# DanielPS555/Radix-sort-Merge-Sort-CUDA---Lab-y-practicos-GPGPU-2023

Hardware: NVIDIA B200
Metric: 32-bit keys sorted/sec at n=2^28 (higher is better)
Workload: dtype int32

## Files before the change

### radix-sort-merge-sort-cuda---lab-y-practicos-gpgpu-2023_b200/csrc/radix.cu

```cuda
#include "radix.cuh"
#include "radix_hist.cuh"
#include "radix_tile.cuh"
#include "radix_pipelined.cuh"
#include "radix_tma.cuh"
#include "radix_tma2.cuh"
#include "radix_tma3.cuh"
#include "radix_misc.cuh"
#include "radix_small.cuh"

#include <atomic>
#include <cstdlib>
#include <mutex>

namespace b200sort {

__global__ void __launch_bounds__(kSmallThreads, 1)
radix_small_kernel(const int32_t *in, int32_t *out, uint32_t n)
{
    radix_small_body<0>(in, out, n, SignXor{0x80000000u, 0x80000000u});
}
__global__ void __launch_bounds__(kSmallThreads, 1)
radix_small_keys_kernel(const int32_t *in, int32_t *out, uint32_t n, SignXor order)
{
    radix_small_body<1>(in, out, n, order);
}

namespace {

using OnesweepFn = void (*)(const int32_t *, int32_t *, int32_t *, size_t, int, RadixControl *,
                            uint32_t *, uint32_t *, int);

struct Variant {
    const char *name;
    int mode;
    int cluster;
    int two_level;
    int threads;
    int tile;
    size_t smem;
// ... 238 lines not shown
    const size_t chunks = div_up(div_up(n, 4), (size_t)kHistThreads * kHistUnroll);
    size_t g = chunks < (size_t)kNumSMs * kHistBlocksPerSM ? chunks : (size_t)kNumSMs * kHistBlocksPerSM;
    return (int)(g < 1 ? 1 : g);
}

}

namespace {
int effective_variant() {
    const int v = g_variant.load();
    if (kVariants[v].mode == kRankAdd && !atomic_order_ok()) return kFallbackVariant;
    return v;
}
}

int radix_set_phase_debug(long long *d_buf) {
    B200_CUDA_TRY(cudaMemcpyToSymbol(g_phase_dbg, &d_buf, sizeof d_buf));
    return B200SORT_OK;
}
int radix_atomic_order_ok() { return atomic_order_ok(); }
unsigned long long radix_check_failures(unsigned long long *per_site) { return tu_check_failures(per_site); }
int radix_num_variants() { return kNumVariants; }
const char *radix_variant_name(int v) { return (v >= 0 && v < kNumVariants) ? kVariants[v].name : nullptr; }
int radix_set_variant(int v) {
    if (v < 0 || v >= kNumVariants) return B200SORT_ERR_INVALID;
    g_variant.store(v);
    g_small_enabled.store((v == 0 && g_small_env_on) ? 1 : 0);
    return B200SORT_OK;
}
void radix_set_skip(int enabled) { g_skip_enabled.store(enabled ? 1 : 0); }
size_t radix_current_tile() { return (size_t)kVariants[g_variant.load()].tile; }
const char *radix_effective_variant_name() { return kVariants[effective_variant()].name; }

size_t radix_workspace_bytes(size_t n) {
    const size_t tiles = div_up(n > 0 ? n : 1, kRadixMinTile);
    const size_t rows = tiles + div_up(tiles, (size_t)kPPGroup) + 1;
    return kRadixControlBytes + 2 * rows * kRadixBins * sizeof(uint32_t);
}

int radix_histogram(const int32_t *d_keys, size_t n, uint32_t *d_hist, cudaStream_t s) {
    RadixControl *scratch = nullptr;
    B200_CUDA_TRY(cudaMallocAsync(reinterpret_cast<void **>(&scratch), kRadixControlBytes, s));
    int rc = ensure_hist_attr();
    if (rc == B200SORT_OK) rc = record_cuda(cudaMemsetAsync(scratch, 0, kRadixZeroBytes, s));
    if (rc == B200SORT_OK && n > 0) {
        radix_histogram_kernel<<<hist_grid(n), kHistThreads, kHistSmemBytes, s>>>(d_keys, n, scratch, nullptr, 0, 0, 0);
        ++g_launch_count;
        rc = record_cuda(cudaGetLastError());
    }
    if (rc == B200SORT_OK)
        rc = record_cuda(cudaMemcpyAsync(d_hist, scratch->hist, sizeof(uint32_t) * kRadixPasses * kRadixBins,
                                         cudaMemcpyDeviceToDevice, s));
    cudaFreeAsync(scratch, s);
    return rc;
}

static int check_ws(void *d_ws, size_t ws_bytes, size_t n) {
    if (d_ws == nullptr || (reinterpret_cast<uintptr_t>(d_ws) & 255) != 0) return B200SORT_ERR_WORKSPACE;
    if (ws_bytes < radix_workspace_bytes(n)) return B200SORT_ERR_WORKSPACE;
    return B200SORT_OK;
}

int radix_single_pass(const int32_t *d_in, int32_t *d_out, size_t n, int pass, void *d_ws,
                      size_t ws_bytes, cudaStream_t s) {
    if (pass < 0 || pass >= kRadixPasses) return B200SORT_ERR_INVALID;
    if (n == 0) return B200SORT_OK;
    B200_TRY(check_ws(d_ws, ws_bytes, n));
    const int v = effective_variant();
    B200_TRY(ensure_smem_attr(v));
    B200_TRY(ensure_hist_attr());
// ... 50 lines not shown
        if (order != nullptr) {
            B200_CUDA_TRY(cudaFuncSetAttribute(reinterpret_cast<const void *>(radix_small_keys_kernel),
                                               cudaFuncAttributeMaxDynamicSharedMemorySize, (int)kSmallSmemBytes));
            radix_small_keys_kernel<<<1, kSmallThreads, kSmallSmemBytes, s>>>(d_in, d_out, (uint32_t)n, *order);
        } else {
            B200_CUDA_TRY(cudaFuncSetAttribute(reinterpret_cast<const void *>(radix_small_kernel),
                                               cudaFuncAttributeMaxDynamicSharedMemorySize, (int)kSmallSmemBytes));
            radix_small_kernel<<<1, kSmallThreads, kSmallSmemBytes, s>>>(d_in, d_out, (uint32_t)n);
        }
        B200_LAUNCH_CHECK();
        return B200SORT_OK;
    }
    int v = effective_variant();
    if (d_n != nullptr && kVariants[v].fn_devn == nullptr) v = atomic_order_ok() ? 0 : kFallbackVariant;
    if (v == 0 && n < kDefaultMinKeys) v = kSmallTileVariant;
    const bool keys = order != nullptr;
    if (keys && (d_n != nullptr || kVariants[v].fn_key == nullptr)) return B200SORT_ERR_INVALID;
    B200_TRY(ensure_smem_attr(v, keys));
    if (d_n != nullptr)
        B200_CUDA_TRY(cudaFuncSetAttribute(reinterpret_cast<const void *>(kVariants[v].fn_devn),
                                           cudaFuncAttributeMaxDynamicSharedMemorySize, (int)kVariants[v].smem));
    B200_TRY(ensure_hist_attr(keys));
    const Variant &var = kVariants[v];
    auto *ctl = static_cast<RadixControl *>(d_ws);
    const size_t tiles = div_up(n, (size_t)var.tile);
    const size_t rows = status_rows(var, tiles);
    uint32_t *status[2];
    status[0] = reinterpret_cast<uint32_t *>(static_cast<unsigned char *>(d_ws) + kRadixControlBytes);
    status[1] = status[0] + rows * kRadixBins;
    const int skip = g_skip_enabled.load();
    const uint32_t in_place = (d_in == d_out) ? 1u : 0u;
    StepTimer timer{s, ms};

    B200_CUDA_TRY(cudaMemsetAsync(ctl, 0, kRadixZeroBytes, s));
    B200_TRY(timer.begin());
    if (d_hist != nullptr) {
        B200_CUDA_TRY(cudaMemsetAsync(status[0], 0, rows * kRadixBins * sizeof(uint32_t), s));
        radix_plan_kernel<<<1, kHistThreads, 0, s>>>(d_hist, d_n, ctl, (uint32_t)skip, in_place);
    } else if (keys) {
        radix_histogram_keys_kernel<<<hist_grid(n), kHistThreads, kHistSmemBytes, s>>>(d_in, n, ctl, status[0],
                                                                                       rows * kRadixBins, (uint32_t)skip,
                                                                                       in_place, *order);
    } else {
        radix_histogram_kernel<<<hist_grid(n), kHistThreads, kHistSmemBytes, s>>>(d_in, n, ctl, status[0], rows * kRadixBins,
                                                                     (uint32_t)skip, in_place, d_n);
    }
    B200_LAUNCH_CHECK();
    B200_TRY(timer.mark());
    for (int pass = 0; pass < kRadixPasses; ++pass) {
        uint32_t *cur = status[pass & 1];
        uint32_t *next = (pass + 1 < kRadixPasses) ? status[(pass + 1) & 1] : nullptr;
        B200_TRY(launch_onesweep(var, tiles, s, d_in, d_out, d_tmp, n, pass, ctl, cur, next, 1, d_n != nullptr, keys));
        B200_TRY(timer.mark());
    }
    if (skip) {
        const size_t blocks = div_up(div_up(n, 4), 256);
        const unsigned grid = (unsigned)(blocks < (size_t)kNumSMs * 8 ? blocks : (size_t)kNumSMs * 8);
        radix_final_copy_kernel<<<grid, 256, 0, s>>>(d_in, d_out, d_tmp, n, ctl, d_n ? 1u : 0u);
        B200_LAUNCH_CHECK();
    }
    B200_TRY(timer.mark());
    return timer.finish();
}

}

int radix_sort(const int32_t *d_in, int32_t *d_out, int32_t *d_tmp, size_t n, void *d_ws,
               size_t ws_bytes, cudaStream_t s, const SignXor *order) {
    return radix_sort_impl(d_in, d_out, d_tmp, n, d_ws, ws_bytes, s, nullptr, nullptr, nullptr, order);
}

int radix_sort_devn(const int32_t *d_in, int32_t *d_out, int32_t *d_tmp, size_t n_max, const uint32_t *d_n,
                    const uint32_t *d_hist, void *d_ws, size_t ws_bytes, cudaStream_t s) {
    if (d_n == nullptr) return B200SORT_ERR_INVALID;
    return radix_sort_impl(d_in, d_out, d_tmp, n_max, d_ws, ws_bytes, s, nullptr, d_n, d_hist);
}

template <int IPT, int SAFE, int KEYS = 0>
int launch_pairs_passes(const int32_t *d_in, int32_t *d_out, int32_t *d_tmp, const int32_t *v_in, int32_t *v_out,
                        int32_t *v_tmp, size_t n, RadixControl *ctl, uint32_t *const *status, cudaStream_t s) {
    constexpr size_t smem = Pipelined2Shape<IPT, 1, 1>::kSmemBytes;
    B200_CUDA_TRY(cudaFuncSetAttribute(reinterpret_cast<const void *>(radix_onesweep_pairs_kernel<IPT, SAFE, KEYS>),
                                       cudaFuncAttributeMaxDynamicSharedMemorySize, (int)smem));
    const size_t tiles = div_up(n, (size_t)Pipelined2Shape<IPT, 1, 1>::kTile);
    const unsigned slots = 2u * kNumSMs;
// ... 78 lines not shown
```

### radix-sort-merge-sort-cuda---lab-y-practicos-gpgpu-2023_b200/csrc/radix_hist.cuh

```cuda
#pragma once
#include "radix.cuh"
#include "radix_async.cuh"

#include <cooperative_groups.h>

namespace cg = cooperative_groups;

namespace b200sort {

constexpr int kHistThreads = 512;
constexpr int kHistUnroll  = 4;
constexpr int kHistBlocksPerSM = 3;
constexpr int kHistSmemWords  = (kRadixPasses / 2) * kRadixBins * 32;
constexpr size_t kHistSmemBytes = (size_t)kHistSmemWords * 4;
constexpr int kHistFlushIters = 128;

__device__ __forceinline__ void hist_add(uint32_t col_s, int32_t key) {
    const uint32_t k = (uint32_t)key;
    const uint32_t d0 = __byte_perm(k, 0u, 0x4440u), d1 = __byte_perm(k, 0u, 0x4441u), d2 = __byte_perm(k, 0u, 0x4442u),
                   d3 = __byte_perm(k, 0u, 0x4443u);
    asm volatile("red.shared.add.u32 [%0], 1;"           :: "r"(col_s + (d0 << 7)) : "memory");
    asm volatile("red.shared.add.u32 [%0], 65536;"       :: "r"(col_s + (d1 << 7)) : "memory");
    asm volatile("red.shared.add.u32 [%0+32768], 1;"     :: "r"(col_s + (d2 << 7)) : "memory");
    asm volatile("red.shared.add.u32 [%0+32768], 65536;" :: "r"(col_s + (d3 << 7)) : "memory");
// ... 134 lines not shown
        bool ok[kHistUnroll];
#pragma unroll
        for (int u = 0; u < kHistUnroll; ++u) {
            const size_t idx = base + (size_t)u * kHistThreads + tid;
            ok[u] = idx < nvec;
            if (ok[u]) r[u] = ld_stream_v4(v + idx);
        }
#pragma unroll
        for (int u = 0; u < kHistUnroll; ++u) {
            if (ok[u]) {
                add(r[u].x); add(r[u].y);
                add(r[u].z); add(r[u].w);
            }
        }
        if (++iters == kHistFlushIters) { hist_flush(sh, ctl, tid); iters = 0; }
    }
    if (blockIdx.x == 0) {
        for (size_t i = tid; i < head; i += kHistThreads) add(keys[i]);
        for (size_t i = tail_start + tid; i < n; i += kHistThreads) add(keys[i]);
    }
    hist_flush(sh, ctl, tid);

    __threadfence();
    __syncthreads();
    if (tid == 0) s_is_last = (atomicAdd(&ctl->hist_blocks_done, 1u) == gridDim.x - 1) ? 1u : 0u;
    if (tid < kRadixPasses) { s_skip[tid] = 0; s_hot[tid] = 0; }
    __syncthreads();
    if (!s_is_last) return;
    __threadfence();

    radix_finish_plan(ctl, n, skip_enabled, in_place, tid, s_warp_sums, s_skip, s_hot);
}

__global__ void __launch_bounds__(kHistThreads)
radix_histogram_kernel(const int32_t *__restrict__ keys, size_t n, RadixControl *ctl,
                       uint32_t *status_to_zero, size_t status_words, uint32_t skip_enabled,
                       uint32_t in_place, const uint32_t *d_n = nullptr)
{
    radix_histogram_body<0>(keys, n, ctl, status_to_zero, status_words, skip_enabled, in_place, d_n,
                            SignXor{0x80000000u, 0x80000000u});
}
__global__ void __launch_bounds__(kHistThreads)
radix_histogram_keys_kernel(const int32_t *__restrict__ keys, size_t n, RadixControl *ctl, uint32_t *status_to_zero,
                            size_t status_words, uint32_t skip_enabled, uint32_t in_place, SignXor order)
{
    radix_histogram_body<1>(keys, n, ctl, status_to_zero, status_words, skip_enabled, in_place, nullptr, order);
}

}
```

### radix-sort-merge-sort-cuda---lab-y-practicos-gpgpu-2023_b200/csrc/radix_tma3.cuh

```cuda
#pragma once
#include "radix_tma2.cuh"

namespace b200sort {

constexpr int kT3StageWords = kT2Tile + kRadixBins * 7 + 64;
constexpr int kT3Group = 4;
constexpr int kT3Win1 = 10;
constexpr int kT3Win2 = 7;
constexpr size_t kT3SmemBytes =
    (size_t)kT3StageWords * 4
    + (size_t)2 * kT2Rows * kRadixBins * 4
    + (size_t)8 * kRadixBins * 4
    + (size_t)(kT3Win1 + kT3Win2) * kRadixBins * 4
    + 256;
static_assert(kT3SmemBytes <= 115712, "two CTAs per SM");

template <int ROWS>
__device__ __forceinline__ void load_window(const uint32_t *win, uint32_t have, uint32_t (&w)[ROWS]) {
    const uint32_t *nearest = win + (size_t)(have - 1) * kRadixBins;
#pragma unroll
    for (int j = 0; j < ROWS; ++j) w[j] = ((uint32_t)j < have) ? nearest[-j * kRadixBins] : 0u;
}
template <int ROWS, int W>
__device__ __forceinline__ uint32_t sum_window(const uint32_t (&w)[ROWS], uint32_t have, const uint32_t *first, uint32_t max_dist) {
    uint32_t acc = 0;
#pragma unroll
    for (int j = 0; j < ROWS; ++j) {
        if ((uint32_t)j < have) {
            uint32_t x = w[j];
            while ((x & ~kValueMask) == 0) x = ld_relaxed_gpu(first - (size_t)j * kRadixBins);
            acc += x & kValueMask;
            if ((x & ~kValueMask) == kFlagIncl) return acc;
        }
    }
    if (max_dist > have) acc += walk_back<W>(first - (size_t)have * kRadixBins, max_dist - have);
    return acc;
}

template <int TIMING, int DEVN = 0, int INSTEP = 0, int ACOUNT = 0, int KEYS = 0>
__device__ __forceinline__ void
radix_onesweep_tma3_body(const int32_t *in_buf, int32_t *out_buf, int32_t *tmp_buf, size_t n, int pass,
                         RadixControl *ctl, uint32_t *status_cur, uint32_t *status_next, int follow_plan)
{
    constexpr int kTile = kT2Tile;
    constexpr int kRows = kT2Rows;
    constexpr uint32_t kNone = 0xFFFFFFFFu;

    extern __shared__ __align__(128) unsigned char smem_tma3[];
    int32_t  *s_stage  = reinterpret_cast<int32_t *>(smem_tma3);
    uint32_t *s_table  = reinterpret_cast<uint32_t *>(s_stage + kT3StageWords);
    uint2    *s_rg     = reinterpret_cast<uint2 *>(s_table + 2 * kRows * kRadixBins);
    uint32_t *s_ptot   = reinterpret_cast<uint32_t *>(s_rg + 2 * kRadixBins);
    uint32_t *s_pin    = s_ptot + 2 * kRadixBins;
    uint32_t *s_win1   = s_pin + 2 * kRadixBins;
    uint32_t *s_win2   = s_win1 + kT3Win1 * kRadixBins;
    uint32_t *s_misc   = s_win2 + kT3Win2 * kRadixBins;
    const uint32_t tid = threadIdx.x, lane = tid & 31, warp = tid >> 5;

    const int32_t *in = in_buf;
    int32_t *out = out_buf;
    if (follow_plan) {
        if (ctl->skip[pass]) {
            const size_t n_now = DEVN ? (size_t)ctl->n_dev : n;
            const size_t tl = (n_now + kTile - 1) / kTile;
            const size_t rows = tl + (tl + kLookGroup - 1) / kLookGroup;
            if (status_next != nullptr)
                for (size_t row = blockIdx.x; row < rows; row += gridDim.x)
                    if (tid < kRadixBins) status_next[row * kRadixBins + tid] = 0;
            return;
// ... 29 lines not shown
        s_misc[8] = atomicAdd(&ctl->ticket[pass], 1u);
        mbar_init(mbar, 1);
        asm volatile("fence.mbarrier_init.release.cluster;" ::: "memory");
        const uint32_t n32 = DEVN ? ctl->n_dev : (uint32_t)n;
        s_misc[20] = n32;
        s_misc[21] = (uint32_t)(((size_t)n32 + kTile - 1) / kTile);
    }
    asm volatile("tcgen05.fence::before_thread_sync;" ::: "memory");
    __syncthreads();
    asm volatile("tcgen05.fence::after_thread_sync;" ::: "memory");
    auto n_f = [&]() -> size_t { return DEVN ? (size_t)reinterpret_cast<volatile uint32_t *>(s_misc)[20] : n; };
    auto tiles_f = [&]() -> size_t { return (size_t)reinterpret_cast<volatile uint32_t *>(s_misc)[21]; };
    const uint32_t tmem_base = s_misc[10];
    const uint32_t tmem_warp = tmem_base + (((warp & 3u) * 32u) << 16) + (warp >> 2) * 64u;

    int32_t ka[kT2Batch], kb[kT2Batch];
    auto load_batch_of = [&](uint32_t t, uint32_t wsel, int batch, int32_t (&k)[kT2Batch]) {
        const size_t tile_base = (size_t)t * kTile;
        const size_t n_now = n_f();
        const uint32_t valid = (n_now - tile_base < (size_t)kTile) ? (uint32_t)(n_now - tile_base) : (uint32_t)kTile;
        const uint32_t o = wsel * (32 * kT2Ipt) + lane + batch * (32 * kT2Batch);
        const int32_t *src = in + tile_base + o;
        if (valid == (uint32_t)kTile) {
#pragma unroll
            for (int i = 0; i < kT2Batch; ++i) k[i] = ld_stream(src + i * 32);
        } else {
#pragma unroll
            for (int i = 0; i < kT2Batch; ++i)
                k[i] = (o + i * 32 < valid) ? ld_stream(src + i * 32) : (KEYS ? (int32_t)ctl->key_pad : 0x7FFFFFFF);
        }
    };
    auto load_batch = [&](uint32_t t, int batch, int32_t (&k)[kT2Batch]) { load_batch_of(t, warp, batch, k); };
    auto sweep = [&](const int32_t (&k)[kT2Batch], uint32_t *wt, bool count_only) {
        const uint32_t d0 = dig(k[0]);
        const uint32_t agree = __ballot_sync(0xffffffffu, d0 == __shfl_sync(0xffffffffu, d0, 0));
        const uint32_t hot_word = follow_plan ? ctl->hot[pass] : 0u;
        const bool hot = hot_word != 0 || __popc(agree) >= 8;
        if (!hot) {
            uint32_t pos[kT2Batch];
#pragma unroll
            for (int i = 0; i < kT2Batch; ++i) {
                uint32_t d = dig(k[i]);
                if (count_only && i >= 2 * kT3Group && i % kT3Group == 0) d += pos[i - kT3Group - 1] >> 31;
                pos[i] = atomicAdd(wt + d, 1u << sh);
                if (!count_only && i >= kT3Group && i % kT3Group == kT3Group - 1) {
#pragma unroll
                    for (int j = i - 2 * kT3Group + 1; j <= i - kT3Group; ++j) {
                        const uint32_t q = (pos[j] >> sh) & 0xffffu;
                        B200_CHECK_AT(11, q < (uint32_t)kT3StageWords);
                        s_stage[q] = k[j];
                    }
                }
            }
            if (!count_only) {
#pragma unroll
                for (int j = kT2Batch - kT3Group; j < kT2Batch; ++j) {
                    const uint32_t q = (pos[j] >> sh) & 0xffffu;
                    B200_CHECK_AT(11, q < (uint32_t)kT3StageWords);
                    s_stage[q] = k[j];
                }
            }
        } else {
#pragma unroll
            for (int i = 0; i < kT2Batch; ++i) {
                const uint32_t d = dig(k[i]);
                const uint32_t hd = hot_word ? hot_word - 1u : __shfl_sync(0xffffffffu, d, 0);
                const bool same = (d == hd);
                const uint32_t sm = __ballot_sync(0xffffffffu, same);
                const uint32_t leader = (uint32_t)(__ffs(sm) - 1) & 31u;
                uint32_t r = 0;
                if (!same || lane == leader)
                    r = (atomicAdd(wt + d, (same ? (uint32_t)__popc(sm) : 1u) << sh) >> sh) & 0xffffu;
                const uint32_t r0 = __shfl_sync(0xffffffffu, r, leader);
                if (same) r = r0 + __popc(sm & lt);
                if (!count_only) {
                    B200_CHECK_AT(11, r < (uint32_t)kT3StageWords);
                    s_stage[r] = k[i];
                }
            }
        }
    };

    auto count_and_park = [&](uint32_t t, uint32_t cb, uint32_t *tab_cur) {
        load_batch(t, 1, kb);
        uint32_t *wt = tab_cur + (warp >> 1) * kRadixBins;
        sweep(ka, wt, true);
        tmem_st16(tmem_warp + cb * 32u, ka);
        sweep(kb, wt, true);
        tmem_st16(tmem_warp + cb * 32u + 16u, kb);
    };
    auto count_and_park_both = [&](uint32_t t, uint32_t cb, uint32_t *tab_cur) {
        uint32_t *wt = tab_cur + (warp >> 1) * kRadixBins;
        const uint32_t tm = tmem_warp + cb * 32u;
        load_batch(t, 1, kb);
        sweep(ka, wt, true);
        tmem_st16(tm, ka);
        tmem_wait_st();
        load_batch_of(t, warp + 8, 0, ka);
        sweep(kb, wt, true);
        tmem_st16(tm + 16u, kb);
        tmem_wait_st();
        load_batch_of(t, warp + 8, 1, kb);
        sweep(ka, wt + 4 * kRadixBins, true);
        tmem_st16(tm + 128u, ka);
        sweep(kb, wt + 4 * kRadixBins, true);
        tmem_st16(tm + 128u + 16u, kb);
        tmem_wait_st();
        asm volatile("tcgen05.fence::before_thread_sync;" ::: "memory");
    };
    auto stage_own = [&](uint32_t cb, uint32_t *tab_prev) {
        const uint32_t tp = tmem_warp + (cb ^ 1) * 32u;
        uint32_t *wt = tab_prev + (warp >> 1) * kRadixBins;
        tmem_wait_st();
// ... 195 lines not shown
        } else if (in_a) {
            if (have_cur) count_and_park(tile, cb, tab_cur);
            B200_STAMP(1);
            bulk_wait_read_all();
            bar_sync(11, kT2Threads);
            B200_STAMP(2);
            if (have_prev) stage_own(cb, tab_prev);
            B200_STAMP(3);
            bar_sync(12, kT2Threads);
            B200_STAMP(4);
            publish();
            B200_STAMP(5);
        } else {
            resolve();
            B200_STAMP(1);
            __threadfence_block();
            bar_arrive(11, kT2Threads);
            B200_STAMP(2);
            if (have_cur) count_and_park(tile, cb, tab_cur);
            B200_STAMP(3);
            bar_sync(12, kT2Threads);
            B200_STAMP(4);
            if (have_prev) stage_own(cb, tab_prev);
            B200_STAMP(5);
        }
        __syncthreads();
        B200_STAMP(6);
        const uint32_t next = s_misc[8];
        if (ACOUNT) {
            if (in_a) {
                if (next < tiles_f()) load_batch(next, 0, ka);
            } else {
                if (tid == kRadixBins && have_cur) request_rows(tile);
                if (have_prev) {
                    const uint2 rg = s_rg[(cb ^ 1) * kRadixBins + bd];
                    const uint32_t start = rg.x & 0xffffu, c = rg.x >> 16, g = rg.y;
                    uint32_t head = (4u - (g & 3u)) & 3u;
                    if (head > c) head = c;
                    const uint32_t body = (c - head) & ~3u;
                    const uint32_t tail = c - head - body;
                    B200_CHECK_AT(13, body == 0 || (((g + head) & 3u) == 0 && ((start + head) & 3u) == 0));
                    B200_CHECK_AT(14, (size_t)g - gmis + c <= n_f() && start + c <= (uint32_t)kT3StageWords);
                    int32_t e[6];
#pragma unroll
                    for (int j = 0; j < 3; ++j) {
                        e[j]     = ((uint32_t)j < head) ? s_stage[start + j] : 0;
                        e[3 + j] = ((uint32_t)j < tail) ? s_stage[start + head + body + j] : 0;
                    }
                    if (body > 0) bulk_store(out_al + g + head, stage_s + (start + head) * 4u, body * 4u);
                    bulk_commit();
#pragma unroll
                    for (int j = 0; j < 3; ++j) {
                        if ((uint32_t)j < head) st_stream(out_al + g + j, e[j]);
                        if ((uint32_t)j < tail) st_stream(out_al + g + head + body + j, e[3 + j]);
                    }
                }
            }
        } else {
            if (next < tiles_f()) load_batch(next, 0, ka);
            if (have_prev) {
                const uint2 rg = s_rg[(cb ^ 1) * kRadixBins + (in_a ? tid : bd)];
                const uint32_t start = rg.x & 0xffffu, c = rg.x >> 16, g = rg.y;
                uint32_t head = (4u - (g & 3u)) & 3u;
                if (head > c) head = c;
                const uint32_t body = (c - head) & ~3u;
                if (in_a) {
                    B200_CHECK_AT(13, body == 0 || (((g + head) & 3u) == 0 && ((start + head) & 3u) == 0));
                    B200_CHECK_AT(14, (size_t)g - gmis + c <= n_f() && start + c <= (uint32_t)kT3StageWords);
                    if (body > 0) bulk_store(out_al + g + head, stage_s + (start + head) * 4u, body * 4u);
                    bulk_commit();
                }
                const uint32_t cnt = in_a ? head : c - head - body;
                const uint32_t first = in_a ? 0u : head + body;
                int32_t e[3];
    #pragma unroll
                for (int j = 0; j < 3; ++j) e[j] = ((uint32_t)j < cnt) ? s_stage[start + first + j] : 0;
    #pragma unroll
                for (int j = 0; j < 3; ++j)
                    if ((uint32_t)j < cnt) st_stream(out_al + g + first + j, e[j]);
            }
            if (!INSTEP && tid == kRadixBins && have_cur) request_rows(tile);
        }
        B200_STAMP(7);
        if (TIMING && g_phase_dbg != nullptr && lane == 0 && (warp == 0 || warp == 8))
            g_phase_dbg[((size_t)dbg_tile * 2 + (warp >> 3)) * 16 + 9] = dbg_tile;
        prev_tile = have_cur ? tile : kNone;
        tile = next;
        ++iter;
    }
// ... 16 lines not shown
```

Before: 105.2 billion.

## Precompute first-pass per-tile digit offsets in histogram, drop decoupled lookback

The histogram kernel now also records per-tile, per-slice digit counts for the lowest digit. A scan kernel turns those into global per-tile prefixes, so the first onesweep pass can scatter without decoupled lookback by reading precomputed offsets. A dedicated first-pass kernel is added, and the sweep and write-run code is factored into shared helpers. The cost is extra workspace, extra global table traffic and one more kernel launch, in exchange for removing serial lookback latency in pass 0.

```diff
diff --git a/radix-sort-merge-sort-cuda---lab-y-practicos-gpgpu-2023_b200/csrc/radix.cu b/radix-sort-merge-sort-cuda---lab-y-practicos-gpgpu-2023_b200/csrc/radix.cu
--- a/radix-sort-merge-sort-cuda---lab-y-practicos-gpgpu-2023_b200/csrc/radix.cu
+++ b/radix-sort-merge-sort-cuda---lab-y-practicos-gpgpu-2023_b200/csrc/radix.cu
@@ -5,6 +5,7 @@
 #include "radix_tma.cuh"
 #include "radix_tma2.cuh"
 #include "radix_tma3.cuh"
+#include "radix_first_pass.cuh"
 #include "radix_misc.cuh"
 #include "radix_small.cuh"
 
@@ -309,10 +310,22 @@
 size_t radix_current_tile() { return (size_t)kVariants[g_variant.load()].tile; }
 const char *radix_effective_variant_name() { return kVariants[effective_variant()].name; }
 
+namespace {
+size_t first_pass_ctas(size_t tiles) { return tiles < (size_t)kHistCountMaxCtas ? tiles : (size_t)kHistCountMaxCtas; }
+size_t first_pass_bytes(size_t n) {
+    const size_t tiles = div_up(n > 0 ? n : 1, (size_t)kT2Tile);
+    const size_t rows = tiles + div_up(tiles, (size_t)kLookGroup);
+    const size_t words = 2 * rows * kRadixBins + tiles * (kFirstTableWords + kRadixBins) + first_pass_ctas(tiles) * kRadixBins;
+    return kRadixControlBytes + words * sizeof(uint32_t);
+}
+}
+
 size_t radix_workspace_bytes(size_t n) {
     const size_t tiles = div_up(n > 0 ? n : 1, kRadixMinTile);
     const size_t rows = tiles + div_up(tiles, (size_t)kPPGroup) + 1;
-    return kRadixControlBytes + 2 * rows * kRadixBins * sizeof(uint32_t);
+    const size_t bytes = kRadixControlBytes + 2 * rows * kRadixBins * sizeof(uint32_t);
+    const size_t first = first_pass_bytes(n);
+    return bytes > first ? bytes : first;
 }
 
 int radix_histogram(const int32_t *d_keys, size_t n, uint32_t *d_hist, cudaStream_t s) {
@@ -429,9 +442,33 @@
     const uint32_t in_place = (d_in == d_out) ? 1u : 0u;
     StepTimer timer{s, ms};
 
+    const bool first = d_n == nullptr && d_hist == nullptr && (v == 0 || v == 3);
+    FirstPassTables ft{};
+    if (first) {
+        ft.slice = status[1] + rows * kRadixBins;
+        ft.prefix = ft.slice + tiles * kFirstTableWords;
+        ft.cta = ft.prefix + tiles * kRadixBins;
+        ft.ctas = (uint32_t)first_pass_ctas(tiles);
+        B200_CUDA_TRY(cudaFuncSetAttribute(keys ? reinterpret_cast<const void *>(radix_histogram_count_keys_kernel)
+                                                : reinterpret_cast<const void *>(radix_histogram_count_kernel),
+                                           cudaFuncAttributeMaxDynamicSharedMemorySize, (int)kHistCountSmemBytes));
+        B200_CUDA_TRY(cudaFuncSetAttribute(keys ? reinterpret_cast<const void *>(radix_first_pass_kernel<1>)
+                                                : reinterpret_cast<const void *>(radix_first_pass_kernel<0>),
+                                           cudaFuncAttributeMaxDynamicSharedMemorySize, (int)kFirstSmemBytes));
+    }
+
     B200_CUDA_TRY(cudaMemsetAsync(ctl, 0, kRadixZeroBytes, s));
     B200_TRY(timer.begin());
-    if (d_hist != nullptr) {
+    if (first) {
+        if (keys)
+            radix_histogram_count_keys_kernel<<<ft.ctas, kHistThreads, kHistCountSmemBytes, s>>>(d_in, n, ctl, (uint32_t)skip,
+                                                                                               in_place, *order, ft);
+        else
+            radix_histogram_count_kernel<<<ft.ctas, kHistThreads, kHistCountSmemBytes, s>>>(d_in, n, ctl, (uint32_t)skip,
+                                                                                         in_place, ft);
+        B200_LAUNCH_CHECK();
+        radix_first_scan_kernel<<<kRadixBins / kFirstScanWarps, kFirstScanWarps * 32, 0, s>>>(ctl, ft);
+    } else if (d_hist != nullptr) {
         B200_CUDA_TRY(cudaMemsetAsync(status[0], 0, rows * kRadixBins * sizeof(uint32_t), s));
         radix_plan_kernel<<<1, kHistThreads, 0, s>>>(d_hist, d_n, ctl, (uint32_t)skip, in_place);
     } else if (keys) {
@@ -447,7 +484,14 @@
     for (int pass = 0; pass < kRadixPasses; ++pass) {
         uint32_t *cur = status[pass & 1];
         uint32_t *next = (pass + 1 < kRadixPasses) ? status[(pass + 1) & 1] : nullptr;
-        B200_TRY(launch_onesweep(var, tiles, s, d_in, d_out, d_tmp, n, pass, ctl, cur, next, 1, d_n != nullptr, keys));
+        if (first && pass == 0) {
+            const unsigned grid = (unsigned)(tiles < (size_t)2 * kNumSMs ? tiles : (size_t)2 * kNumSMs);
+            if (keys) radix_first_pass_kernel<1><<<grid, kT2Threads, kFirstSmemBytes, s>>>(d_in, d_out, d_tmp, n, ctl, next, ft);
+            else      radix_first_pass_kernel<0><<<grid, kT2Threads, kFirstSmemBytes, s>>>(d_in, d_out, d_tmp, n, ctl, next, ft);
+            B200_LAUNCH_CHECK();
+        } else {
+            B200_TRY(launch_onesweep(var, tiles, s, d_in, d_out, d_tmp, n, pass, ctl, cur, next, 1, d_n != nullptr, keys));
+        }
         B200_TRY(timer.mark());
     }
     if (skip) {
diff --git a/radix-sort-merge-sort-cuda---lab-y-practicos-gpgpu-2023_b200/csrc/radix_first_pass.cuh b/radix-sort-merge-sort-cuda---lab-y-practicos-gpgpu-2023_b200/csrc/radix_first_pass.cuh
--- /dev/null
+++ b/radix-sort-merge-sort-cuda---lab-y-practicos-gpgpu-2023_b200/csrc/radix_first_pass.cuh
@@ -0,0 +1,146 @@
+#pragma once
+#include "radix_tma3.cuh"
+
+namespace b200sort {
+
+static_assert(kFirstTile == kT2Tile && kFirstSlice == 32 * kT2Ipt && kFirstRows == kT2Rows, "one slice per warp");
+
+constexpr size_t kFirstSmemBytes =
+    (size_t)kT3StageWords * 4
+    + (size_t)kT2Rows * kRadixBins * 4
+    + (size_t)kRadixBins * 8
+    + 64;
+static_assert(kFirstSmemBytes <= 115712, "two CTAs per SM");
+
+template <int KEYS>
+__global__ void __launch_bounds__(kT2Threads, 2)
+radix_first_pass_kernel(const int32_t *in_buf, int32_t *out_buf, int32_t *tmp_buf, size_t n, RadixControl *ctl,
+                        uint32_t *status_next, FirstPassTables ft)
+{
+    constexpr int kTile = kT2Tile;
+    constexpr int kRows = kT2Rows;
+    extern __shared__ __align__(128) unsigned char smem_first[];
+    int32_t  *s_stage = reinterpret_cast<int32_t *>(smem_first);
+    uint32_t *s_table = reinterpret_cast<uint32_t *>(s_stage + kT3StageWords);
+    uint2    *s_rg    = reinterpret_cast<uint2 *>(s_table + kRows * kRadixBins);
+    uint32_t *s_wsum  = reinterpret_cast<uint32_t *>(s_rg + kRadixBins);
+    const uint32_t tid = threadIdx.x, lane = tid & 31, warp = tid >> 5;
+
+    const size_t tiles = (n + kTile - 1) / kTile;
+    const size_t rows = tiles + (tiles + kLookGroup - 1) / kLookGroup;
+    if (ctl->skip[0]) {
+        for (size_t row = blockIdx.x; row < rows; row += gridDim.x)
+            if (tid < kRadixBins) status_next[row * kRadixBins + tid] = 0;
+        return;
+    }
+    for (size_t row = tiles + blockIdx.x; row < rows; row += gridDim.x)
+        if (tid < kRadixBins) status_next[row * kRadixBins + tid] = 0;
+    const int32_t *in = (ctl->src_sel[0] == kSelIn) ? in_buf : (ctl->src_sel[0] == kSelTmp) ? tmp_buf : out_buf;
+    int32_t *out = (ctl->dst_sel[0] == kSelTmp) ? tmp_buf : out_buf;
+    const uint32_t flips = KEYS ? flips_of(ctl->key_neg, ctl->key_pos, 0) : 0u;
+    auto dig = [&](int32_t k) -> uint32_t { return KEYS ? digit_of_image(k, 0, flips) : digit_of(k, 0, 0u); };
+    const uint32_t hot_word = ctl->hot[0];
+    const uint32_t lt = lanemask_lt();
+    const uint32_t sh = (warp & 1) * 16;
+    const uint32_t gmis = (uint32_t)((reinterpret_cast<uintptr_t>(out) >> 2) & 3u);
+    int32_t *out_al = out - gmis;
+    const uint32_t stage_s = smem_u32(s_stage);
+    uint32_t *wt = s_table + (warp >> 1) * kRadixBins;
+
+    int32_t ka[kT2Batch], kb[kT2Batch];
+    auto load = [&](size_t t) {
+        const size_t tile_base = t * kTile;
+        const uint32_t valid = (n - tile_base < (size_t)kTile) ? (uint32_t)(n - tile_base) : (uint32_t)kTile;
+        const uint32_t o = warp * (32 * kT2Ipt) + lane;
+        const int32_t *src = in + tile_base + o;
+        if (valid == (uint32_t)kTile) {
+#pragma unroll
+            for (int i = 0; i < kT2Batch; ++i) { ka[i] = ld_stream(src + i * 32); kb[i] = ld_stream(src + (kT2Batch + i) * 32); }
+        } else {
+            const int32_t pad = KEYS ? (int32_t)ctl->key_pad : 0x7FFFFFFF;
+#pragma unroll
+            for (int i = 0; i < kT2Batch; ++i) {
+                ka[i] = (o + i * 32 < valid) ? ld_stream(src + i * 32) : pad;
+                kb[i] = (o + (kT2Batch + i) * 32 < valid) ? ld_stream(src + (kT2Batch + i) * 32) : pad;
+            }
+        }
+    };
+    auto prefetch = [&](size_t t) {
+        if (t < tiles) {
+            const size_t left = (n - t * kTile) * 4;
+            const uintptr_t a0 = reinterpret_cast<uintptr_t>(in + t * kTile) & ~(uintptr_t)15;
+            const uint32_t bytes = (uint32_t)((left < (size_t)kTile * 4 ? left : (size_t)kTile * 4) & ~(size_t)15);
+            if (bytes > 0) bulk_prefetch_l2(reinterpret_cast<const void *>(a0), bytes);
+        }
+    };
+
+    size_t t = blockIdx.x;
+    if (tid == 0) prefetch(t + gridDim.x);
+    if (t < tiles) load(t);
+    for (; t < tiles; t += gridDim.x) {
+        if (tid < kRadixBins) {
+            uint32_t c[kRows];
+            const uint32_t *sc = ft.slice + t * kFirstTableWords + tid;
+#pragma unroll
+            for (int r = 0; r < kRows; ++r) c[r] = __ldcs(sc + r * kRadixBins);
+            const uint32_t g0 = __ldcg(&ft.cta[(size_t)first_pass_owner(t, tiles, ft.ctas) * kRadixBins + tid])
+                              + __ldcs(&ft.prefix[t * kRadixBins + tid]);
+            status_next[t * kRadixBins + tid] = 0;
+            uint32_t real = 0;
+#pragma unroll
+            for (int r = 0; r < kRows; ++r) real += (c[r] & 0xffffu) + (c[r] >> 16);
+            const size_t valid = n - t * kTile;
+            uint32_t total = real;
+            if (valid < (size_t)kTile && tid == kRadixBins - 1) {
+#pragma unroll
+                for (int r = 0; r < kRows; ++r) {
+                    uint32_t p[2];
+#pragma unroll
+                    for (int h = 0; h < 2; ++h) {
+                        const size_t end = (size_t)(2 * r + h + 1) * kFirstSlice;
+                        const size_t pad = end > valid ? end - valid : 0;
+                        p[h] = (uint32_t)(pad < (size_t)kFirstSlice ? pad : (size_t)kFirstSlice);
+                    }
+                    c[r] += p[0] | (p[1] << 16);
+                    total += p[0] + p[1];
+                }
+            }
+            const uint32_t slot = ((total + 3u) & ~3u) + 4u;
+            uint32_t x = slot;
+#pragma unroll
+            for (int o = 1; o < 32; o <<= 1) {
+                const uint32_t y = __shfl_up_sync(0xffffffffu, x, o);
+                if (lane >= (uint32_t)o) x += y;
+            }
+            if (lane == 31) s_wsum[warp] = x;
+            bulk_wait_read_all();
+            bar_sync(1, kRadixBins);
+            uint32_t add = 0;
+#pragma unroll
+            for (int w = 0; w < 8; ++w) add += (w < (int)warp) ? s_wsum[w] : 0u;
+            const uint32_t g = g0 + gmis;
+            B200_CHECK_AT(12, (size_t)g0 + real <= n);
+            const uint32_t start = x - slot + add + (g & 3u);
+            uint32_t run = start;
+#pragma unroll
+            for (int r = 0; r < kRows; ++r) {
+                const uint32_t lo = c[r] & 0xffffu;
+                s_table[r * kRadixBins + tid] = run | ((run + lo) << 16);
+                run += lo + (c[r] >> 16);
+            }
+            s_rg[tid] = make_uint2(start | (real << 16), g);
+        }
+        __syncthreads();
+        t3_sweep(ka, wt, false, dig, hot_word, s_stage, lane, lt, sh);
+        t3_sweep(kb, wt, false, dig, hot_word, s_stage, lane, lt, sh);
+        fence_proxy_async_smem();
+        __syncthreads();
+        const size_t next = t + gridDim.x;
+        if (tid == 0) prefetch(next + gridDim.x);
+        if (next < tiles) load(next);
+        if (tid < kRadixBins) t3_write_run(s_stage, stage_s, out_al, s_rg[tid], n, gmis);
+    }
+    bulk_wait_all();
+}
+
+}
diff --git a/radix-sort-merge-sort-cuda---lab-y-practicos-gpgpu-2023_b200/csrc/radix_hist.cuh b/radix-sort-merge-sort-cuda---lab-y-practicos-gpgpu-2023_b200/csrc/radix_hist.cuh
--- a/radix-sort-merge-sort-cuda---lab-y-practicos-gpgpu-2023_b200/csrc/radix_hist.cuh
+++ b/radix-sort-merge-sort-cuda---lab-y-practicos-gpgpu-2023_b200/csrc/radix_hist.cuh
@@ -190,6 +190,204 @@
     radix_finish_plan(ctl, n, skip_enabled, in_place, tid, s_warp_sums, s_skip, s_hot);
 }
 
+constexpr int kFirstTile   = 16384;
+constexpr int kFirstSlice  = 1024;
+constexpr int kFirstRows   = kFirstTile / kFirstSlice / 2;
+constexpr int kFirstTableWords = kFirstRows * kRadixBins;
+constexpr size_t kHistCountSmemBytes = kHistSmemBytes + (size_t)kFirstTableWords * 4;
+constexpr int kHistCountMaxCtas = kNumSMs * kHistBlocksPerSM;
+constexpr int kHistCountFlushTiles = 64;
+
+struct FirstPassTables {
+    uint32_t *slice;
+    uint32_t *prefix;
+    uint32_t *cta;
+    uint32_t ctas;
+};
+
+__device__ __forceinline__ uint32_t first_pass_owner(size_t t, size_t tiles, uint32_t ctas) {
+    return (uint32_t)(((t + 1) * ctas - 1) / tiles);
+}
+
+__device__ __forceinline__ void hist_add_upper(uint32_t col_s, uint32_t k) {
+    const uint32_t d1 = __byte_perm(k, 0u, 0x4441u), d2 = __byte_perm(k, 0u, 0x4442u), d3 = __byte_perm(k, 0u, 0x4443u);
+    asm volatile("red.shared.add.u32 [%0], 65536;"       :: "r"(col_s + (d1 << 7)) : "memory");
+    asm volatile("red.shared.add.u32 [%0+32768], 1;"     :: "r"(col_s + (d2 << 7)) : "memory");
+    asm volatile("red.shared.add.u32 [%0+32768], 65536;" :: "r"(col_s + (d3 << 7)) : "memory");
+}
+
+template <int KEYS>
+__device__ __forceinline__ void
+radix_histogram_count_body(const int32_t *__restrict__ keys, size_t n, RadixControl *ctl, uint32_t skip_enabled,
+                           uint32_t in_place, SignXor order, FirstPassTables ft)
+{
+    extern __shared__ __align__(16) uint32_t sh[];
+    uint32_t *s_tab = sh + kHistSmemWords;
+    __shared__ uint32_t s_warp_sums[kRadixBins / 32];
+    __shared__ uint32_t s_skip[kRadixPasses];
+    __shared__ uint32_t s_hot[kRadixPasses];
+    __shared__ uint32_t s_is_last;
+
+    const uint32_t tid = threadIdx.x, lane = tid & 31;
+    if (KEYS && blockIdx.x == 0 && tid == 0) {
+        ctl->key_neg = order.neg;
+        ctl->key_pos = order.pos;
+        ctl->key_pad = key_of_last_image(order);
+    }
+    const uint32_t xneg = order.neg ^ 0x80000000u, xpos = order.pos ^ 0x80000000u;
+    {
+        uint4 *z = reinterpret_cast<uint4 *>(sh);
+        for (uint32_t i = tid; i < (kHistSmemWords + kFirstTableWords) / 4; i += kHistThreads) z[i] = make_uint4(0, 0, 0, 0);
+    }
+    __syncthreads();
+
+    const uint32_t col = smem_u32(sh + lane);
+    const uint32_t tab_s = smem_u32(s_tab);
+    auto img = [&](int32_t k) -> uint32_t { return KEYS ? sign_xor((uint32_t)k, xneg, xpos) : (uint32_t)k; };
+    auto add_one = [&](uint32_t k, uint32_t i) {
+        hist_add_upper(col, k);
+        const uint32_t s = i >> 10;
+        B200_CHECK_AT(11, s < 2u * kFirstRows);
+        asm volatile("red.shared.add.u32 [%0], %1;" :: "r"(tab_s + (((s >> 1) * kRadixBins + (k & 255u)) << 2)),
+                     "r"(1u << ((s & 1u) * 16)) : "memory");
+    };
+    auto add_hot = [&](uint32_t k, uint32_t i, bool ok) {
+        if (ok) hist_add_upper(col, k);
+        const uint32_t s = i >> 10, d = k & 255u;
+        const uint32_t hd = __shfl_sync(0xffffffffu, d, 0), hs = __shfl_sync(0xffffffffu, s, 0);
+        const bool same = ok && d == hd && s == hs;
+        const uint32_t sm = __ballot_sync(0xffffffffu, same);
+        if (same ? lane == (uint32_t)(__ffs(sm) - 1) : ok) {
+            B200_CHECK_AT(11, s < 2u * kFirstRows);
+            asm volatile("red.shared.add.u32 [%0], %1;" :: "r"(tab_s + (((s >> 1) * kRadixBins + d) << 2)),
+                         "r"((same ? (uint32_t)__popc(sm) : 1u) << ((s & 1u) * 16)) : "memory");
+        }
+    };
+
+    const size_t tiles = (n + kFirstTile - 1) / kFirstTile;
+    const size_t t_end = tiles * (blockIdx.x + 1) / gridDim.x;
+    uint32_t run = 0;
+    int since_flush = 0;
+    for (size_t t = tiles * blockIdx.x / gridDim.x; t < t_end; ++t) {
+        const int32_t *tk = keys + t * kFirstTile;
+        const uint32_t cnt = (n - t * kFirstTile < (size_t)kFirstTile) ? (uint32_t)(n - t * kFirstTile) : (uint32_t)kFirstTile;
+        if (tid == 0 && t + 1 < t_end) {
+            const size_t left = (n - (t + 1) * kFirstTile) * 4;
+            const uintptr_t a0 = reinterpret_cast<uintptr_t>(tk + kFirstTile) & ~(uintptr_t)15;
+            const uint32_t bytes = (uint32_t)((left < (size_t)kFirstTile * 4 ? left : (size_t)kFirstTile * 4) & ~(size_t)15);
+            if (bytes > 0) bulk_prefetch_l2(reinterpret_cast<const void *>(a0), bytes);
+        }
+        uint32_t head = (uint32_t)(((16 - (reinterpret_cast<uintptr_t>(tk) & 15)) & 15) / 4);
+        if (head > cnt) head = cnt;
+        const uint32_t nvec = (cnt - head) / 4;
+        const int4 *v = reinterpret_cast<const int4 *>(tk + head);
+        for (uint32_t base = 0; base < (uint32_t)kFirstTile / 4; base += kHistThreads * kHistUnroll) {
+            int4 r[kHistUnroll];
+            bool ok[kHistUnroll];
+#pragma unroll
+            for (int u = 0; u < kHistUnroll; ++u) {
+                const uint32_t idx = base + u * kHistThreads + tid;
+                ok[u] = idx < nvec;
+                if (ok[u]) r[u] = ld_stream_v4(v + idx);
+            }
+            const uint32_t d0 = ok[0] ? img(r[0].x) & 255u : 0u;
+            const uint32_t hd0 = __shfl_sync(0xffffffffu, d0, 0);
+            const uint32_t agree = __ballot_sync(0xffffffffu, ok[0] && d0 == hd0);
+            if (__popc(agree) < 8) {
+#pragma unroll
+                for (int u = 0; u < kHistUnroll; ++u) {
+                    if (ok[u]) {
+                        const uint32_t i = head + 4 * (base + u * kHistThreads + tid);
+                        add_one(img(r[u].x), i);     add_one(img(r[u].y), i + 1);
+                        add_one(img(r[u].z), i + 2); add_one(img(r[u].w), i + 3);
+                    }
+                }
+            } else {
+#pragma unroll
+                for (int u = 0; u < kHistUnroll; ++u) {
+                    const uint32_t i = head + 4 * (base + u * kHistThreads + tid);
+                    add_hot(img(r[u].x), i, ok[u]);     add_hot(img(r[u].y), i + 1, ok[u]);
+                    add_hot(img(r[u].z), i + 2, ok[u]); add_hot(img(r[u].w), i + 3, ok[u]);
+                }
+            }
+        }
+        const uint32_t tail_start = head + nvec * 4;
+        if (tid < head) add_one(img(tk[tid]), tid);
+        else if (tid >= 32 && tid - 32 < cnt - tail_start) add_one(img(tk[tail_start + tid - 32]), tail_start + tid - 32);
+        __syncthreads();
+        if (tid < kRadixBins) {
+            uint32_t *dst = ft.slice + t * kFirstTableWords + tid;
+            uint32_t tot = 0;
+#pragma unroll
+            for (int r = 0; r < kFirstRows; ++r) {
+                const uint32_t c = s_tab[r * kRadixBins + tid];
+                s_tab[r * kRadixBins + tid] = 0;
+                st_stream(reinterpret_cast<int32_t *>(dst + r * kRadixBins), (int32_t)c);
+                tot += (c & 0xffffu) + (c >> 16);
+            }
+            ft.prefix[t * kRadixBins + tid] = run;
+            run += tot;
+        }
+        __syncthreads();
+        if (++since_flush == kHistCountFlushTiles) { hist_flush(sh, ctl, tid); since_flush = 0; }
+    }
+    hist_flush(sh, ctl, tid);
+    if (tid < kRadixBins) {
+        ft.cta[(size_t)blockIdx.x * kRadixBins + tid] = run;
+        if (run) atomicAdd(&ctl->hist[0][tid], run);
+    }
+
+    __threadfence();
+    __syncthreads();
+    if (tid == 0) s_is_last = (atomicAdd(&ctl->hist_blocks_done, 1u) == gridDim.x - 1) ? 1u : 0u;
+    if (tid < kRadixPasses) { s_skip[tid] = 0; s_hot[tid] = 0; }
+    __syncthreads();
+    if (!s_is_last) return;
+    __threadfence();
+
+    radix_finish_plan(ctl, n, skip_enabled, in_place, tid, s_warp_sums, s_skip, s_hot);
+}
+
+__global__ void __launch_bounds__(kHistThreads, kHistBlocksPerSM)
+radix_histogram_count_kernel(const int32_t *__restrict__ keys, size_t n, RadixControl *ctl, uint32_t skip_enabled,
+                             uint32_t in_place, FirstPassTables ft)
+{
+    radix_histogram_count_body<0>(keys, n, ctl, skip_enabled, in_place, SignXor{0x80000000u, 0x80000000u}, ft);
+}
+__global__ void __launch_bounds__(kHistThreads, kHistBlocksPerSM)
+radix_histogram_count_keys_kernel(const int32_t *__restrict__ keys, size_t n, RadixControl *ctl, uint32_t skip_enabled,
+                                  uint32_t in_place, SignXor order, FirstPassTables ft)
+{
+    radix_histogram_count_body<1>(keys, n, ctl, skip_enabled, in_place, order, ft);
+}
+
+constexpr int kFirstScanWarps = 8;
+__global__ void __launch_bounds__(kFirstScanWarps * 32)
+radix_first_scan_kernel(const RadixControl *ctl, FirstPassTables ft)
+{
+    constexpr int kPerLane = (kHistCountMaxCtas + 31) / 32;
+    const uint32_t lane = threadIdx.x & 31, d = blockIdx.x * kFirstScanWarps + (threadIdx.x >> 5);
+    uint32_t v[kPerLane];
+#pragma unroll
+    for (int j = 0; j < kPerLane; ++j) {
+        const uint32_t c = j * 32 + lane;
+        v[j] = c < ft.ctas ? __ldcg(&ft.cta[(size_t)c * kRadixBins + d]) : 0u;
+    }
+    uint32_t carry = __ldcg(&ctl->base[0][d]);
+#pragma unroll
+    for (int j = 0; j < kPerLane; ++j) {
+        uint32_t x = v[j];
+#pragma unroll
+        for (int o = 1; o < 32; o <<= 1) {
+            const uint32_t y = __shfl_up_sync(0xffffffffu, x, o);
+            if (lane >= (uint32_t)o) x += y;
+        }
+        const uint32_t c = j * 32 + lane;
+        if (c < ft.ctas) ft.cta[(size_t)c * kRadixBins + d] = carry + x - v[j];
+        carry += __shfl_sync(0xffffffffu, x, 31);
+    }
+}
+
 __global__ void __launch_bounds__(kHistThreads)
 radix_histogram_kernel(const int32_t *__restrict__ keys, size_t n, RadixControl *ctl,
                        uint32_t *status_to_zero, size_t status_words, uint32_t skip_enabled,
diff --git a/radix-sort-merge-sort-cuda---lab-y-practicos-gpgpu-2023_b200/csrc/radix_tma3.cuh b/radix-sort-merge-sort-cuda---lab-y-practicos-gpgpu-2023_b200/csrc/radix_tma3.cuh
--- a/radix-sort-merge-sort-cuda---lab-y-practicos-gpgpu-2023_b200/csrc/radix_tma3.cuh
+++ b/radix-sort-merge-sort-cuda---lab-y-practicos-gpgpu-2023_b200/csrc/radix_tma3.cuh
@@ -35,6 +35,81 @@
     }
     if (max_dist > have) acc += walk_back<W>(first - (size_t)have * kRadixBins, max_dist - have);
     return acc;
+}
+
+template <class Dig>
+__device__ __forceinline__ void t3_sweep(const int32_t (&k)[kT2Batch], uint32_t *wt, bool count_only, const Dig &dig,
+                                         uint32_t hot_word, int32_t *s_stage, uint32_t lane, uint32_t lt, uint32_t sh) {
+    const uint32_t d0 = dig(k[0]);
+    const uint32_t agree = __ballot_sync(0xffffffffu, d0 == __shfl_sync(0xffffffffu, d0, 0));
+    const bool hot = hot_word != 0 || __popc(agree) >= 8;
+    if (!hot) {
+        uint32_t pos[kT2Batch];
+#pragma unroll
+        for (int i = 0; i < kT2Batch; ++i) {
+            uint32_t d = dig(k[i]);
+            if (count_only && i >= 2 * kT3Group && i % kT3Group == 0) d += pos[i - kT3Group - 1] >> 31;
+            pos[i] = atomicAdd(wt + d, 1u << sh);
+            if (!count_only && i >= kT3Group && i % kT3Group == kT3Group - 1) {
+#pragma unroll
+                for (int j = i - 2 * kT3Group + 1; j <= i - kT3Group; ++j) {
+                    const uint32_t q = (pos[j] >> sh) & 0xffffu;
+                    B200_CHECK_AT(11, q < (uint32_t)kT3StageWords);
+                    s_stage[q] = k[j];
+                }
+            }
+        }
+        if (!count_only) {
+#pragma unroll
+            for (int j = kT2Batch - kT3Group; j < kT2Batch; ++j) {
+                const uint32_t q = (pos[j] >> sh) & 0xffffu;
+                B200_CHECK_AT(11, q < (uint32_t)kT3StageWords);
+                s_stage[q] = k[j];
+            }
+        }
+    } else {
+#pragma unroll
+        for (int i = 0; i < kT2Batch; ++i) {
+            const uint32_t d = dig(k[i]);
+            const uint32_t hd = hot_word ? hot_word - 1u : __shfl_sync(0xffffffffu, d, 0);
+            const bool same = (d == hd);
+            const uint32_t sm = __ballot_sync(0xffffffffu, same);
+            const uint32_t leader = (uint32_t)(__ffs(sm) - 1) & 31u;
+            uint32_t r = 0;
+            if (!same || lane == leader)
+                r = (atomicAdd(wt + d, (same ? (uint32_t)__popc(sm) : 1u) << sh) >> sh) & 0xffffu;
+            const uint32_t r0 = __shfl_sync(0xffffffffu, r, leader);
+            if (same) r = r0 + __popc(sm & lt);
+            if (!count_only) {
+                B200_CHECK_AT(11, r < (uint32_t)kT3StageWords);
+                s_stage[r] = k[i];
+            }
+        }
+    }
+}
+
+__device__ __forceinline__ void t3_write_run(const int32_t *s_stage, uint32_t stage_s, int32_t *out_al, uint2 rg,
+                                             size_t n, uint32_t gmis) {
+    const uint32_t start = rg.x & 0xffffu, c = rg.x >> 16, g = rg.y;
+    uint32_t head = (4u - (g & 3u)) & 3u;
+    if (head > c) head = c;
+    const uint32_t body = (c - head) & ~3u;
+    const uint32_t tail = c - head - body;
+    B200_CHECK_AT(13, body == 0 || (((g + head) & 3u) == 0 && ((start + head) & 3u) == 0));
+    B200_CHECK_AT(14, (size_t)g - gmis + c <= n && start + c <= (uint32_t)kT3StageWords);
+    int32_t e[6];
+#pragma unroll
+    for (int j = 0; j < 3; ++j) {
+        e[j]     = ((uint32_t)j < head) ? s_stage[start + j] : 0;
+        e[3 + j] = ((uint32_t)j < tail) ? s_stage[start + head + body + j] : 0;
+    }
+    if (body > 0) bulk_store(out_al + g + head, stage_s + (start + head) * 4u, body * 4u);
+    bulk_commit();
+#pragma unroll
+    for (int j = 0; j < 3; ++j) {
+        if ((uint32_t)j < head) st_stream(out_al + g + j, e[j]);
+        if ((uint32_t)j < tail) st_stream(out_al + g + head + body + j, e[3 + j]);
+    }
 }
 
 template <int TIMING, int DEVN = 0, int INSTEP = 0, int ACOUNT = 0, int KEYS = 0>
@@ -130,53 +205,7 @@
     };
     auto load_batch = [&](uint32_t t, int batch, int32_t (&k)[kT2Batch]) { load_batch_of(t, warp, batch, k); };
     auto sweep = [&](const int32_t (&k)[kT2Batch], uint32_t *wt, bool count_only) {
-        const uint32_t d0 = dig(k[0]);
-        const uint32_t agree = __ballot_sync(0xffffffffu, d0 == __shfl_sync(0xffffffffu, d0, 0));
-        const uint32_t hot_word = follow_plan ? ctl->hot[pass] : 0u;
-        const bool hot = hot_word != 0 || __popc(agree) >= 8;
-        if (!hot) {
-            uint32_t pos[kT2Batch];
-#pragma unroll
-            for (int i = 0; i < kT2Batch; ++i) {
-                uint32_t d = dig(k[i]);
-                if (count_only && i >= 2 * kT3Group && i % kT3Group == 0) d += pos[i - kT3Group - 1] >> 31;
-                pos[i] = atomicAdd(wt + d, 1u << sh);
-                if (!count_only && i >= kT3Group && i % kT3Group == kT3Group - 1) {
-#pragma unroll
-                    for (int j = i - 2 * kT3Group + 1; j <= i - kT3Group; ++j) {
-                        const uint32_t q = (pos[j] >> sh) & 0xffffu;
-                        B200_CHECK_AT(11, q < (uint32_t)kT3StageWords);
-                        s_stage[q] = k[j];
-                    }
-                }
-            }
-            if (!count_only) {
-#pragma unroll
-                for (int j = kT2Batch - kT3Group; j < kT2Batch; ++j) {
-                    const uint32_t q = (pos[j] >> sh) & 0xffffu;
-                    B200_CHECK_AT(11, q < (uint32_t)kT3StageWords);
-                    s_stage[q] = k[j];
-                }
-            }
-        } else {
-#pragma unroll
-            for (int i = 0; i < kT2Batch; ++i) {
-                const uint32_t d = dig(k[i]);
-                const uint32_t hd = hot_word ? hot_word - 1u : __shfl_sync(0xffffffffu, d, 0);
-                const bool same = (d == hd);
-                const uint32_t sm = __ballot_sync(0xffffffffu, same);
-                const uint32_t leader = (uint32_t)(__ffs(sm) - 1) & 31u;
-                uint32_t r = 0;
-                if (!same || lane == leader)
-                    r = (atomicAdd(wt + d, (same ? (uint32_t)__popc(sm) : 1u) << sh) >> sh) & 0xffffu;
-                const uint32_t r0 = __shfl_sync(0xffffffffu, r, leader);
-                if (same) r = r0 + __popc(sm & lt);
-                if (!count_only) {
-                    B200_CHECK_AT(11, r < (uint32_t)kT3StageWords);
-                    s_stage[r] = k[i];
-                }
-            }
-        }
+        t3_sweep(k, wt, count_only, dig, follow_plan ? ctl->hot[pass] : 0u, s_stage, lane, lt, sh);
     };
 
     auto count_and_park = [&](uint32_t t, uint32_t cb, uint32_t *tab_cur) {
@@ -438,29 +467,7 @@
                 if (next < tiles_f()) load_batch(next, 0, ka);
             } else {
                 if (tid == kRadixBins && have_cur) request_rows(tile);
-                if (have_prev) {
-                    const uint2 rg = s_rg[(cb ^ 1) * kRadixBins + bd];
-                    const uint32_t start = rg.x & 0xffffu, c = rg.x >> 16, g = rg.y;
-                    uint32_t head = (4u - (g & 3u)) & 3u;
-                    if (head > c) head = c;
-                    const uint32_t body = (c - head) & ~3u;
-                    const uint32_t tail = c - head - body;
-                    B200_CHECK_AT(13, body == 0 || (((g + head) & 3u) == 0 && ((start + head) & 3u) == 0));
-                    B200_CHECK_AT(14, (size_t)g - gmis + c <= n_f() && start + c <= (uint32_t)kT3StageWords);
-                    int32_t e[6];
-#pragma unroll
-                    for (int j = 0; j < 3; ++j) {
-                        e[j]     = ((uint32_t)j < head) ? s_stage[start + j] : 0;
-                        e[3 + j] = ((uint32_t)j < tail) ? s_stage[start + head + body + j] : 0;
-                    }
-                    if (body > 0) bulk_store(out_al + g + head, stage_s + (start + head) * 4u, body * 4u);
-                    bulk_commit();
-#pragma unroll
-                    for (int j = 0; j < 3; ++j) {
-                        if ((uint32_t)j < head) st_stream(out_al + g + j, e[j]);
-                        if ((uint32_t)j < tail) st_stream(out_al + g + head + body + j, e[3 + j]);
-                    }
-                }
+                if (have_prev) t3_write_run(s_stage, stage_s, out_al, s_rg[(cb ^ 1) * kRadixBins + bd], n_f(), gmis);
             }
         } else {
             if (next < tiles_f()) load_batch(next, 0, ka);
```

Result: slower. 98.29 billion (median of 6 runs) (-6.6%).
